# quocdat32461997/ggpm

Hardware: AMD Instinct MI355X
Metric: HierMPNEncoder fwd+bwd target row (SURVEY 8(d): encoder + KL heads + optimizer, tree fixed-point hint on; full depth loops in full_depth_loops, the full VAE fwd+bwd row in vae_step) of BASELINE's molecules/sec VAE fwd+bwd (hidden=300, depth=20, batch=32) (higher is better)
Workload: dtype f32

## Files before the change

### ggpm_amd/_lib.py

```python
from __future__ import annotations

import ctypes
import os
from ctypes import c_char_p, c_double, c_float, c_int, c_size_t, c_void_p, POINTER

from . import build as _build

_LIB = None

GGPM_OK, GGPM_ERR_ARG, GGPM_ERR_LAUNCH, GGPM_ERR_UNSUPPORTED, GGPM_ERR_WORKSPACE = range(5)

P = c_void_p
I = c_int
SIGNATURES = {
    "ggpm_version": (I, []),
    "ggpm_error_string": (c_char_p, [I]),
    "ggpm_padded_hidden": (I, [I]),
    "ggpm_padded_to_csr": (I, [P, I, I, P, P, P]),
    "ggpm_padded_to_csr_pair": (I, [P, I, I, P, P, P, I, I, P, P, P]),
    "ggpm_csr_transpose": (I, [P, P, I, I, P, P, P, P]),
    "ggpm_extract_column": (I, [P, I, I, I, P, P]),
    "ggpm_gemm_workspace_bytes": (c_size_t, [I, I, I]),
    "ggpm_gemm": (I, [I, I, I, I, I, P, I, P, I, P, I, I, P, I, I, I, P, c_size_t, P]),
    "ggpm_gemm_grouped": (I, [I, I, I, I, I, I, P, P]),
# ... 10 lines not shown
    "ggpm_gemm_form_query": (I, [P, P]),
    "ggpm_act_backward": (I, [P, P, I, I, I, I, I, P, P]),
    "ggpm_segment_sum": (I, [P, I, P, P, I, I, P, I, I, I, P]),
    "ggpm_segment_sum_masked": (I, [I, P, I, P, P, I, I, P, I, P, I, I, P, P, I, I, I, P]),
    "ggpm_gather_rows": (I, [P, I, P, I, I, P, I, I, I, P]),
    "ggpm_scatter_rows": (I, [P, I, P, I, I, P, I, I, P]),
    "ggpm_adam_step": (I, [P, P, P, P, c_size_t, c_float, c_float, c_float, c_float, c_float, I, P]),
    "ggpm_flat_sqnorm_workspace_bytes": (c_size_t, [c_size_t]),
    "ggpm_flat_sqnorm_partials": (I, [P, c_size_t, P, c_size_t, P]),
    "ggpm_flat_norm_finish": (I, [P, I, c_float, P, P]),
    "ggpm_adam_step_groups": (I, [P, P, P, P, c_size_t, P, I, P, I, P, I, c_float, P, I, P]),
    "ggpm_onehot": (I, [P, I, I, P, I, I, I, P]),
    "ggpm_embed_graph": (I, [P, I, P, I, I, I, I, P, I, P, I, P]),
    "ggpm_level_bf16_storage": (I, [I, I]),
    "ggpm_level_form_query": (I, [I, I, I, I, I, P, P]),
    "ggpm_gru_backward_stashes": (I, [P, I, I, I, POINTER(c_void_p), POINTER(c_void_p)]),
    "ggpm_lstm_backward_stashes": (I, [P, I, I, I, POINTER(c_void_p), POINTER(c_void_p), POINTER(c_void_p)]),
    "ggpm_sum_slots": (I, [P, I, c_size_t, P, P]),
    "ggpm_gru_pack_floats": (c_size_t, [I]),
    "ggpm_gru_forward": (I, [I, I, I, P, P, P, P, I, P, I, P, P, I, P, P, P, P, P, P, P, P, P, P, I, P, P]),
    "ggpm_gru_backward_workspace_bytes": (c_size_t, [I, I, I]),
    "ggpm_gru_backward": (I, [I, I, I, P, P, I, P, I, P, I, P, P, P, P, P, P, P, P, P, P, P, P, P, P, P,
                              P, I, P, I, P, P, I, P, c_size_t, I, P, P]),
    "ggpm_gru_weight_grads": (I, [I, I, I, P, P, P, P, c_size_t, P, I, P, I, P, P, I, P, P]),
    "ggpm_gru_sparse_forward": (I, [I, I, I, P, P, P, P, P, P, I, P, I, P, P, I, P, P, P, P, P, P, P, P, P, P, I, P, P]),
    "ggpm_gru_sparse_backward": (I, [I, I, I, P, P, P, I, P, I, P, I, P, P, P, P, P, P, P, P, P, P, P, P, P, P, P, P,
                                     P, I, P, I, P, P, I, P, c_size_t, P, P]),
    "ggpm_weight_grads_stacked_workspace_bytes": (c_size_t, [I, I]),
    "ggpm_gru_weight_grads_stacked": (I, [I, I, I, P, P, P, P, P, P, P, I, P, I, P, P, I, P, c_size_t, P]),
    "ggpm_lstm_weight_grads_stacked": (I, [I, I, I, P, P, P, P, P, P, P, I, P, I, P, I, P, I, P, c_size_t, P]),
# ... 122 lines not shown
```

### ggpm_amd/csrc/encoder.hip

```cpp
#include "common.h"
#include "level_call.h"
#include <condition_variable>
#include <cstdlib>
#include <deque>
#include <functional>
#include <mutex>
#include <thread>

namespace {

struct Arena {
    char* base;
    size_t off;
    bool overflow;
    size_t cap;
    template <typename T>
    T* take(size_t n) {
        const size_t bytes = (n * sizeof(T) + 255) & ~(size_t)255;
        T* p = base ? reinterpret_cast<T*>(base + off) : nullptr;
        off += bytes;
        if (base && off > cap) overflow = true;
        return p;
    }
};

struct Csr {
    int32_t *rowptr, *col;
    int rows, ncols, cap;
    int32_t *rowptrT, *colT, *cursor;
};

struct LevelSaved {
    float *X, *Hs, *Cs, *Qs, *St, *wpack, *nei;
    float* hout;
};

struct Saved {
    Csr gpred, gagr, tpred, tagr, tcgr, tsrc, root, motif, attach;
    int32_t *src, *attr0, *motif_id, *attach_id, *iota;
    float *hnode_a, *hmess_a;
    LevelSaved lv[3];
    float *finput_i, *pooled, *hnode_i, *hmess_i, *finput_t, *hnode_t, *hmess_t, *f, *n;
};

struct Dims {
    int H, Hp, He, Hep, depthT, depthG, atom, n_motif, n_attach;
    int N1g, E1g, Kga, Kgb, N1t, E1t, Kta, Ktb, Ktc, B;
    int ld_n, ld_m, ld_t, Ig, It;
    int lstm, nX;
// ... 40 lines not shown
    c.col = A.take<int32_t>(c.cap);
    c.rowptrT = A.take<int32_t>(ncols + 1);
    c.colT = A.take<int32_t>(c.cap);
    c.cursor = A.take<int32_t>(ncols);
}

void take_level(Arena& A, LevelSaved& L, int E1, int N1, int Hp, int H, int depth, bool lstm) {
    const size_t slot = (size_t)E1 * Hp;
    L.X = A.take<float>(cell_gates(lstm).n * slot);
    L.Hs = A.take<float>((size_t)(depth + 1) * slot);
    L.Cs = lstm ? A.take<float>((size_t)(depth + 1) * slot) : nullptr;
    L.Qs = A.take<float>((size_t)depth * slot);
    L.St = A.take<float>((size_t)5 * depth * slot);
    L.wpack = A.take<float>(ggpm_level_pack_floats(lstm, H));
    L.nei = A.take<float>((size_t)N1 * Hp);
}

void layout_saved(Arena& A, const Dims& d, Saved& s) {
    s.lv[0].hout = s.lv[1].hout = s.lv[2].hout = nullptr;
    take_csr(A, s.gpred, d.E1g, d.E1g, d.E1g * d.Kgb);
    take_csr(A, s.gagr, d.N1g, d.E1g, d.N1g * d.Kga);
    take_csr(A, s.tpred, d.E1t, d.E1t, d.E1t * d.Ktb);
    take_csr(A, s.tagr, d.N1t, d.E1t, d.N1t * d.Kta);
    take_csr(A, s.tcgr, d.N1t, d.N1g, d.N1t * d.Ktc);
    s.src = A.take<int32_t>(d.E1t); s.attr0 = A.take<int32_t>(d.E1t);
    s.motif_id = A.take<int32_t>(d.N1t); s.attach_id = A.take<int32_t>(d.N1t);
    const int nio = (d.E1t > d.N1t ? d.E1t : d.N1t) + 1;
    s.iota = A.take<int32_t>(nio > d.B + 1 ? nio : d.B + 1);
    auto take_index = [&](Csr& c, int rows, int ncols) {
        c.rows = rows; c.ncols = ncols; c.cap = rows;
// ... 2 lines not shown
    };
    take_index(s.tsrc, d.E1t, d.N1t);
    take_index(s.root, d.B, d.N1t);
    take_index(s.motif, d.N1t, d.n_motif);
    take_index(s.attach, d.N1t, d.n_attach);
    s.hnode_a = A.take<float>((size_t)d.N1g * d.ld_n);
    s.hmess_a = A.take<float>((size_t)d.E1g * d.ld_m);
    take_level(A, s.lv[0], d.E1t, d.N1t, d.Hp, d.H, d.depthT, d.lstm);
    take_level(A, s.lv[1], d.E1t, d.N1t, d.Hp, d.H, d.depthT, d.lstm);
    take_level(A, s.lv[2], d.E1g, d.N1g, d.Hp, d.H, d.depthG, d.lstm);
    s.finput_i = A.take<float>((size_t)d.N1t * d.Hep); s.pooled = A.take<float>((size_t)d.N1t * d.Hp);
    s.hnode_i = A.take<float>((size_t)d.N1t * d.Hp); s.hmess_i = A.take<float>((size_t)d.E1t * d.ld_t);
    s.finput_t = A.take<float>((size_t)d.N1t * d.Hep);
    s.hnode_t = A.take<float>((size_t)d.N1t * d.Hp); s.hmess_t = A.take<float>((size_t)d.E1t * d.ld_t);
    s.f = A.take<float>((size_t)d.B * d.Hp); s.n = A.take<float>((size_t)d.B * d.Hp);
}

void take_csr_fwd(Arena& A, Csr& c, int rows, int ncols, int cap) {
    c.rows = rows; c.ncols = ncols; c.cap = cap < 1 ? 1 : cap;
    c.rowptr = A.take<int32_t>(rows + 1);
    c.col = A.take<int32_t>(c.cap);
    c.rowptrT = c.colT = c.cursor = nullptr;
}

void layout_infer(Arena& A, const Dims& d, Saved& s) {
    s = Saved{};
    take_csr_fwd(A, s.gpred, d.E1g, d.E1g, d.E1g * d.Kgb);
    take_csr_fwd(A, s.gagr, d.N1g, d.E1g, d.N1g * d.Kga);
    take_csr_fwd(A, s.tpred, d.E1t, d.E1t, d.E1t * d.Ktb);
    take_csr_fwd(A, s.tagr, d.N1t, d.E1t, d.N1t * d.Kta);
// ... 7 lines not shown
    L.X = A.take<float>((size_t)d.nX * slot);
    L.Hs = A.take<float>(2 * slot);
    L.Qs = A.take<float>(2 * slot);
    L.Cs = d.lstm ? A.take<float>(2 * slot) : nullptr;
    L.hout = A.take<float>(slot);
    L.wpack = A.take<float>(ggpm_level_pack_floats(d.lstm, d.H));
    for (int l = 0; l < 3; ++l) {
        s.lv[l] = L;
        s.lv[l].nei = A.take<float>((size_t)(l == 2 ? d.N1g : d.N1t) * d.Hp);
    }
    s.finput_i = A.take<float>((size_t)d.N1t * d.Hep); s.pooled = A.take<float>((size_t)d.N1t * d.Hp);
    s.hnode_i = A.take<float>((size_t)d.N1t * d.Hp); s.hmess_i = A.take<float>((size_t)d.E1t * d.ld_t);
    s.finput_t = A.take<float>((size_t)d.N1t * d.Hep);
    s.hnode_t = A.take<float>((size_t)d.N1t * d.Hp); s.hmess_t = A.take<float>((size_t)d.E1t * d.ld_t);
    s.f = A.take<float>((size_t)d.B * d.Hp); s.n = A.take<float>((size_t)d.B * d.Hp);
}

__global__ void iota_k(int32_t* out, int n) {
    const int i = blockIdx.x * blockDim.x + threadIdx.x;
    if (i < n) out[i] = i;
}

enum { P_EC = 0, P_EI, P_WC, P_BC, P_WI, P_BI, P_WROOT, P_BROOT, P_LEVEL0 };
enum { L_WO = 0, L_BO, L_WZ, L_BZ, L_WR, L_UR, L_BU, L_WH, L_BH, L_COUNT };
enum { Q_WO = 0, Q_BO, Q_WI, Q_BI, Q_WOG, Q_BOG, Q_WU, Q_BU, Q_WF, Q_BF, Q_COUNT };
struct LevelSlots { int count, w[4], b[4], ur, bu, ld[4]; };
constexpr LevelSlots GRU_SLOTS = {L_COUNT, {L_WZ, L_WR, L_WH, -1}, {L_BZ, -1, L_BH, -1}, L_UR, L_BU, {}};
constexpr LevelSlots LSTM_SLOTS = {Q_COUNT, {Q_WI, Q_WOG, Q_WU, Q_WF}, {Q_BI, Q_BOG, Q_BU, Q_BF}, -1, -1, {}};
inline const LevelSlots& level_slots(bool lstm) { return lstm ? LSTM_SLOTS : GRU_SLOTS; }
inline int lwo(const Dims& d, int level) { return P_LEVEL0 + level * level_slots(d.lstm).count + L_WO; }
// ... 173 lines not shown
    return c;
}

int level_forward(const Dims& d, int E1, int N1, int I, int depth, const float* x, int ldx, float* const* P, int level,
                  const Csr& pred, const Csr& agr, LevelSaved& L, ggpm_stream_t s) {
    const int H = d.H, Hp = d.Hp;
    const size_t slot = (size_t)E1 * Hp;
    const int run = run_steps(d, level, depth, E1);
    const LevelTag tag(level);
    ggpm_level_opts o = level_opts(d);
    o.run_depth = run;
    const bool infer = L.hout != nullptr;
    o.h_out = L.hout;
    const int fs = infer ? 0 : fixed_slot(d, level, depth, E1);
    o.fixed_slot = fs;
    const float* result = infer ? L.hout : L.Hs + (size_t)(fs ? fs : depth) * slot;
    const LevelSlots gs = gate_slots(d.lstm, level, I, H);
    const LevelCall c = level_call(d, E1, I, depth, P, gs, pred, L);
    GgpmGemmProblem gp[4];
    for (int k = 0; k < d.nX; ++k)
        gp[k] = {x, ldx, P[gs.w[k]], gs.ld[k], L.X + k * slot, Hp, Hp, gs.b[k] < 0 ? nullptr : P[gs.b[k]], 0, GGPM_ACT_NONE, 0};
    CK(ggpm_gemm_grouped(0, 1, E1, H, I, d.nX, gp, s));
    CK(ggpm_level_forward(c, !infer, &o, s));
    if (!infer) CK(replicate_tail(d, E1, depth, run, level, L, s));
    CK(ggpm_segment_sum(result, Hp, agr.rowptr, agr.col, N1, H, L.nei, Hp, 0, Hp, s));
    return GGPM_OK;
}

int transpose(const Csr& c, const int32_t* col, ggpm_stream_t s) {
    return ggpm_csr_transpose(c.rowptr, col ? col : c.col, c.rows, c.ncols, c.rowptrT, c.colT, c.cursor, s);
// ... 504 lines not shown
```

### ggpm_amd/csrc/level_host.h

```cpp
#pragma once
#include "tile_mma.h"
#include <cstdlib>
#include <type_traits>

namespace {

constexpr size_t GGPM_LDS_LIMIT = 160 * 1024;

template <typename K>
inline void set_lds(K kernel, size_t bytes) { ggpm_set_lds(kernel, bytes); }

inline bool env_no_fuse_b() { static const bool v = ggpm_dev_env("GGPM_NO_FUSE_B") != nullptr; return v; }
inline bool env_adebug() { static const bool v = ggpm_dev_env("GGPM_ADEBUG") != nullptr; return v; }

inline int pick_tg(int E1, int NT) {
    static const char* const tg_env = ggpm_dev_env("GGPM_TG");
    if (const char* e = tg_env) { int v = atoi(e); if (v >= 1 && v <= 64) return v; }
    static const char* const tg_small_env = ggpm_dev_env("GGPM_TG_SMALL");
    if (const char* e = tg_small_env) {
        int v = atoi(e);
        if (v >= 1 && v <= 64 && (E1 + 15) / 16 <= 64) return v < NT ? v : NT;
    }
    static const char* const tg_large_env = ggpm_dev_env("GGPM_TG_LARGE");
    if (const char* e = tg_large_env) {
// ... 18 lines not shown
    static const bool on = [] { const char* e = ggpm_dev_env("GGPM_GATE_SPLIT"); return !e || atoi(e) != 0; }();
    if (!on || rt2) return 0;
    if (dtype != 3 && (!single_group || sparse)) return 0;
    return Cell::mode2_fits(Hp) ? 2 : 0;
}

struct LevelPlan { int tg; bool rt2; int gm; };
template <class Cell>
inline LevelPlan level_plan(const ggpm_level_opts& o, int E1, int Hp, bool sparse) {
    LevelPlan p;
    p.tg = pick_tg(E1, Hp / 16);
    p.rt2 = Cell::use_rt2(o, E1, Hp, sparse);
    p.gm = gate_mode<Cell>(o, Hp, p.rt2, p.tg >= Hp / 16, sparse);
    return p;
}
struct StepLds { int fuse; size_t a, b; };
inline StepLds step_lds(const StepNeed& need, int max_tiles, int Hp, int tg, bool rt2, int gm, bool may_fuse) {
    const int rows = rt2 ? 32 : 16, NT = Hp / 16;
    const bool split = gm == 2;
    const size_t fused = lds_bytes(need.fused, rows, Hp, split);
    StepLds p;
    p.fuse = (!rt2 && may_fuse && ggpm_ceil_div(NT, tg) == 1 && (!max_tiles || NT <= max_tiles) && fused <= GGPM_LDS_LIMIT &&
              !env_no_fuse_b()) ? 1 : 0;
    p.a = p.fuse ? fused : lds_bytes(need.a, rows, Hp, split);
    p.b = lds_bytes(need.b, rows, Hp, split);
    return p;
}
template <class Cell>
inline StepLds fwd_step(int Hp, int tg, bool rt2, int gm, bool with_b) {
    return step_lds(Cell::fwd, 0, Hp, tg, rt2, gm, with_b);
// ... 159 lines not shown
```

### ggpm_amd/csrc/mpn_gru.hip

```cpp
#include "tile_mma.h"
#include "level_host.h"
#include "level_call.h"
#include <cstdlib>
#include <cstdio>

__global__ void ggpm_pack_weight_kernel(GgpmPackArgs a) {
    const int Hp = a.Hp, H = a.H, KC = Hp / 16;
    const int lane = threadIdx.x;
    const int kc = blockIdx.x, t = blockIdx.y, m = blockIdx.z;
    const float* __restrict__ W = a.W[m];
    const int ldw = a.ldw[m];
    const int out = 16 * t + (lane & 15);
    if (a.bf16 == 2) {
        const int KC32 = ggpm_kc32_dev(Hp);
        float x[8];
#pragma unroll
        for (int i = 0; i < 8; ++i) {
            const int k = 32 * kc + 8 * (lane >> 4) + i;
            x[i] = (out < H && k < H) ? (a.transpose ? W[(size_t)k * ldw + out] : W[(size_t)out * ldw + k]) : 0.f;
        }
        uint2 lo[3], hi[3];
        ggpm_split3(make_float4(x[0], x[1], x[2], x[3]), lo[0], lo[1], lo[2]);
        ggpm_split3(make_float4(x[4], x[5], x[6], x[7]), hi[0], hi[1], hi[2]);
        __bf16* dst = reinterpret_cast<__bf16*>(a.dst) + (size_t)m * 2 * ggpm_packed_matrix_floats(Hp, 2);
// ... 60 lines not shown
    float *Hnew, *Qnew;
    float *S, *G, *Z, *M, *R;
    const float *Wz, *Wh, *Ur;
    const float* bu;
    const int32_t *rowptr, *col;
    int ablate;
    const unsigned char* frozen;
    int fuse_b;
    unsigned long long* dbg;
    int bf16;
    int st16;
    int h0_zero;
    float* Hout;
    const float* src_h;
    const int32_t* src_idx;
};

__global__ void pad_bias(const float* __restrict__ b, int H, int Hp, float* __restrict__ out) {
    const int c = blockIdx.x * blockDim.x + threadIdx.x;
    if (c < Hp) out[c] = (c < H) ? b[c] : 0.f;
}

__device__ __forceinline__ float4 one_minus(float4 r) { return make_float4(1.f - r.x, 1.f - r.y, 1.f - r.z, 1.f - r.w); }

template <bool STASH, int GM, int RTT, bool ST16 = false>
__global__ void GGPM_A_BOUNDS gru_fwd_a(GruFwdArgs a) {
    constexpr int ROWS = RTT * 16;
    constexpr bool BF16 = GM == 1, SPLIT = GM == 2;
    static_assert(!SPLIT || RTT == 1, "split operands: one row tile per workgroup");
    static_assert(!ST16 || GM == 1, "bf16 storage goes with bf16 gate products");
    extern __shared__ __attribute__((aligned(16))) float lds[];
// ... 172 lines not shown
        const float* Th = lds + 2 * ROWS * LD;
        for (int tt = wave; tt < NT; tt += GGPM_NWA) {
            const int c = 16 * tt + 4 * (lane >> 4);
            const float4 b = ggpm_ld4(a.bu + c);
            f32x4 acc[1][1];
            ggpm_zero_acc<1, 1>(acc);
            const float* const tiles[1] = {Th};
            const int tn = tt + GGPM_NWA < NT ? tt + GGPM_NWA : -1;
            if constexpr (SPLIT) {
                const __bf16* const imgs[1] = {Ih};
                ggpm_wave_gemm_split<1>(imgs, PLANE, LDH, wps3, KC32, tt, tn, lane, acc, sring3);
            } else if constexpr (BF16) ggpm_wave_gemm_bf16<1, 1>(tiles, LD, wps3, Hp, tt, lane, acc);
            else ggpm_wave_gemm_ring<1, 1>(tiles, LD, wps3, KC, tt, tn, lane, acc, ring3);
            if (row < a.E1) ggpm_stx<ST16>(a.Qnew, (size_t)row * Hp + c, ggpm_f4(acc[0][0]) + b);
        }
    }
}

template <int GM, int RTT, bool ST16 = false>
__global__ void GGPM_A_BOUNDS gru_fwd_b(GruFwdArgs a) {
    constexpr int ROWS = RTT * 16;
    constexpr bool BF16 = GM == 1, SPLIT = GM == 2;
    static_assert(!SPLIT || RTT == 1, "split operands: one row tile per workgroup");
    extern __shared__ __attribute__((aligned(16))) float lds[];
    const int Hp = a.Hp, LD = Hp + 4, KC = Hp / 16, NT = Hp / 16;
    float* Th = lds;
    const int LDH = ggpm_split_ldh(Hp), PLANE = ROWS * LDH, KC32 = ggpm_kc32_dev(Hp);
    __bf16* Ih = reinterpret_cast<__bf16*>(lds);
    const int lane = threadIdx.x & 63;
    const int wave = __builtin_amdgcn_readfirstlane(threadIdx.x >> 6);
// ... 380 lines not shown
        static const int mode = [] { const char* e = ggpm_dev_env("GGPM_RT2"); return e ? atoi(e) : 1; }();
        if (mode == 0 || sparse) return false;
        if (lds_tiles(2, Hp, 32) > GGPM_LDS_LIMIT) return false;
        return mode == 2 || o.prefer_narrow || ggpm_ceil_div(E1, 16) >= GGPM_RT2_MIN_ROW_TILES;
    }
    static bool mode2_fits(int Hp) { return lds_tiles(1, Hp) + 2 * ggpm_split_image_bytes(16, Hp) <= GGPM_LDS_LIMIT; }
    static bool shape_ok(int, int Hp) { return lds_tiles(2, Hp) <= GGPM_LDS_LIMIT; }
};

inline unsigned long long* adebug_stamps(unsigned long long*& buf) {
    if (!env_adebug()) return nullptr;
    if (!buf) (void)hipMalloc(&buf, 64);
    return buf;
}

void launch_fwd(GruFwdArgs a, bool rt2, bool stash, bool with_b, double flops1, hipStream_t s) {
    const StepLds step = fwd_step<GruCell>(a.Hp, a.tg, rt2, a.bf16, with_b);
    a.fuse_b = step.fuse;
    static unsigned long long* dbg_buf = nullptr;
    static int dbg_count = 0;
    a.dbg = adebug_stamps(dbg_buf);
    ggpm_timing_begin(GruCell::timing_base, s, (step.fuse + (a.h0_zero ? 0 : GruCell::gate_products)) * flops1);
    for_variant<GruCell>(a.st16, rt2, a.bf16, [&](auto GM, auto RTT, auto ST16) {
        launch_step(stash ? gru_fwd_a<true, GM, RTT, ST16> : gru_fwd_a<false, GM, RTT, ST16>, a, rt2, step.a, s);
    });
    ggpm_timing_end(GruCell::timing_base, s);
    if (a.dbg && (++dbg_count % 97) == 0) {
        unsigned long long h[7];
        const dim3 grid = step_grid(a, rt2);
        (void)hipStreamSynchronize(s);
        (void)hipMemcpy(h, a.dbg, sizeof(h), hipMemcpyDeviceToHost);
        fprintf(stderr, "[adebug E1=%d grid=%dx%d fuse=%d] gather %.2f barrier %.2f gemm %.2f epilogue %.2f us; wave 15 starts "
                "+%.2f, gathers %.2f\n", a.E1, grid.x, grid.y, a.fuse_b, (h[1] - h[0]) * 0.01, (h[2] - h[1]) * 0.01,
// ... 36 lines not shown
        ggpm_timing_end(GruCell::timing_base + 5, s);
    }
}

}

extern "C" size_t ggpm_gru_pack_floats(int H) {
    const int Hp = ggpm_padded_hidden(H);
    return 3 * ggpm_packed_matrix_slot(Hp) + (size_t)Hp;
}

int ggpm_gru_level_form(int E1, int H, int sparse, int training, const ggpm_level_opts& o, ggpm_level_form* out) {
    return level_form<GruCell>(E1, H, sparse, training, o, out);
}

namespace {
__global__ void sparse_init_state(const float* __restrict__ h_in, const unsigned char* __restrict__ frozen,
                                  float* __restrict__ H0, int Hp) {
    const int c = blockIdx.x * blockDim.x + threadIdx.x;
    const int r = blockIdx.y;
    if (c >= Hp) return;
    H0[(size_t)r * Hp + c] = frozen[r] ? h_in[(size_t)r * Hp + c] : 0.f;
}
}

int gru_forward_impl(const LevelCall& c, int save_for_backward, const ggpm_level_opts& o, ggpm_stream_t stream) {
    GGPM_CLEAR_STALE_ERROR();
    const int E1 = c.rows, H = c.H, depth = c.depth;
    float *Hs = c.Hs, *Qs = c.Qs, *wpack = c.wpack;
    const unsigned char* frozen = c.frozen;
    bool ok = E1 > 0 && H > 0 && depth > 0 && c.bu && c.pred_rowptr && c.pred_col && Hs && Qs && wpack;
    for (int k = 0; k < 3; ++k) ok = ok && c.X[k] && c.W[k];
    for (int k = 0; k < 5; ++k) ok = ok && (c.St[k] || !save_for_backward);
    if (!ok) return GGPM_ERR_ARG;
    const int Hp = ggpm_padded_hidden(H);
    if (!GruCell::shape_ok(E1, Hp)) return GGPM_ERR_UNSUPPORTED;
    hipStream_t s = (hipStream_t)stream;
    const size_t slot = (size_t)E1 * Hp;
    const LevelPlan plan = level_plan<GruCell>(o, E1, Hp, frozen != nullptr);
    const bool rt2 = plan.rt2;
    const int bf16 = plan.gm;
    const size_t mstep = ggpm_packed_matrix_floats(Hp, bf16);
    float* pWz = wpack; float* pWh = wpack + mstep; float* pUr = wpack + 2 * mstep;
    float* pbu = wpack + 3 * ggpm_packed_matrix_slot(Hp);
    {
        GgpmPackArgs pk = {};
        pk.W[0] = c.W[0]; pk.ldw[0] = c.ldw[0]; pk.W[1] = c.W[2]; pk.ldw[1] = c.ldw[2]; pk.W[2] = c.W[1]; pk.ldw[2] = c.ldw[1];
        pk.H = H; pk.Hp = Hp; pk.transpose = 0; pk.dst = wpack; pk.bias = c.bu; pk.bias_out = pbu; pk.bf16 = bf16;
        if (!o.weights_packed) ggpm_launch_pack(pk, 3, s);
    }
    dim3 ig(ggpm_ceil_div(Hp, 256), E1);
    const int tg0 = plan.tg;
    const bool gathered = o.gather_h && o.gather_idx && frozen;
    if (frozen) {
        if (c.h_in != Hs && !gathered) sparse_init_state<<<ig, 256, 0, s>>>(c.h_in, frozen, Hs, Hp);
        GruFwdArgs a0 = {};
// ... 34 lines not shown
            a.R = c.St[4] + (size_t)(t - 1) * slot;
            if (!stash) a.S = a.G = a.Z = a.M = a.R = nullptr;
        } else if (infer) {
            a.Hprev = ggpm_slot_ptr(Hs, (t - 1) & 1, slot, st16); a.Hnew = ggpm_slot_ptr(Hs, t & 1, slot, st16);
            a.Qprev = ggpm_slot_ptr(Qs, (t - 1) & 1, slot, st16); a.Qnew = ggpm_slot_ptr(Qs, t & 1, slot, st16);
            if (t == run_depth) {
                if (st16) a.Hout = o.h_out;
                else a.Hnew = o.h_out;
            }
            a.S = a.G = a.Z = a.M = a.R = nullptr;
        } else {
            a.Hprev = Hs + (size_t)((t - 1) & 1) * slot; a.Hnew = Hs + (size_t)(t & 1) * slot;
            a.Qprev = Qs + (size_t)((t - 1) & 1) * slot; a.Qnew = Qs + (size_t)(t & 1) * slot;
            a.S = a.G = a.Z = a.M = a.R = nullptr;
        }
        launch_fwd(a, rt2, stash, t < depth, flops1, s);
    }
    GGPM_CHECK_LAUNCH();
    return GGPM_OK;
}

#define GRU_FORWARD_OPERANDS(c) \
    c.rows = E1; c.H = H; c.depth = depth; \
    c.X[0] = Xz; c.X[1] = Xr; c.X[2] = Xh; \
    c.W[0] = Wz_h; c.ldw[0] = ld_wz; c.W[1] = Ur; c.ldw[1] = ld_ur; c.W[2] = Wh_h; c.ldw[2] = ld_wh; c.bu = bu; \
    c.pred_rowptr = pred_rowptr; c.pred_col = pred_col; \
    c.Hs = Hs; c.Qs = Qs; c.St[0] = Ss; c.St[1] = Gs; c.St[2] = Zs; c.St[3] = Ms; c.St[4] = Rs; c.wpack = wpack;
extern "C" int ggpm_gru_forward(int E1, int H, int depth, const float* Xz, const float* Xr, const float* Xh,
                                const float* Wz_h, int ld_wz, const float* Ur, int ld_ur, const float* bu,
                                const float* Wh_h, int ld_wh, const int32_t* pred_rowptr,
                                const int32_t* pred_col, float* Hs, float* Qs, float* Ss, float* Gs, float* Zs,
// ... 307 lines not shown
```

### ggpm_amd/functional.py

```python
from __future__ import annotations

import ctypes
import os
import weakref
from typing import List, Optional, Sequence, Tuple

import torch

from . import _dev, _lib
from .nnutils import version_of
from .parallel import grad_view

ACT_NONE, ACT_RELU, ACT_TANH, ACT_SIGMOID = 0, 1, 2, 3


def _stream() -> ctypes.c_void_p:
    return ctypes.c_void_p(torch._C._cuda_getCurrentRawStream(torch._C._cuda_getDevice()))


def _p(t: Optional[torch.Tensor]) -> ctypes.c_void_p:
    return ctypes.c_void_p(0 if t is None else t.data_ptr())


def _need_gpu(*ts: torch.Tensor) -> None:
# ... 559 lines not shown
        v = list(v) if isinstance(v, (list, tuple)) else [v] * 4
        return _I4(*(v + [0] * (4 - len(v))))
    call = GemmCall(GEMM_ENTRIES.index(entry), ta, tb, M, N, count, four(K), four(lda), four(ldb), four(ldc), four(n_pad),
                    four(base_a), four(base_b), four(base_lo), int(ws_bytes is not None), mode, ws_bytes or 0)
    out = GemmForm()
    _lib.check(_lib.load().ggpm_gemm_form_query(ctypes.byref(call), ctypes.byref(out)), "gemm_form_query")
    return out


class LevelOpts(ctypes.Structure):
    _fields_ = [("gate_dtype", ctypes.c_int), ("prefer_narrow", ctypes.c_int), ("weights_packed", ctypes.c_int),
                ("defer_stash", ctypes.c_void_p * 4), ("gather_h", ctypes.c_void_p), ("gather_c", ctypes.c_void_p),
                ("gather_idx", ctypes.c_void_p), ("scatter_h", ctypes.c_void_p), ("scatter_c", ctypes.c_void_p),
                ("scatter_idx", ctypes.c_void_p), ("skip_x_sums", ctypes.c_int), ("run_depth", ctypes.c_int),
                ("lo", ctypes.c_int), ("skip_bias_u", ctypes.c_int), ("skip_sparse_wgrads", ctypes.c_int),
                ("h_out", ctypes.c_void_p), ("c_out", ctypes.c_void_p), ("fixed_slot", ctypes.c_int)]


class LevelForm(ctypes.Structure):
    _fields_ = [("Hp", ctypes.c_int), ("tiles", ctypes.c_int), ("tg", ctypes.c_int), ("groups", ctypes.c_int),
                ("rt2", ctypes.c_int), ("gate_mode", ctypes.c_int), ("st16", ctypes.c_int), ("fuse_fwd", ctypes.c_int),
                ("fuse_bwd", ctypes.c_int), ("lds_fwd_a", ctypes.c_size_t), ("lds_fwd_b", ctypes.c_size_t),
                ("lds_bwd_a", ctypes.c_size_t), ("lds_bwd_b", ctypes.c_size_t)]


def level_form(lstm: bool, E1: int, H: int, sparse: bool = False, training: bool = True, opts: Optional[LevelOpts] = None):
    out = LevelForm()
    rc = _lib.load().ggpm_level_form_query(int(lstm), E1, H, int(sparse), int(training),
                                           None if opts is None else ctypes.byref(opts), ctypes.byref(out))
    if rc == _lib.GGPM_ERR_UNSUPPORTED:
        return None
# ... 885 lines not shown
```

### include/ggpm_hip.h

```cpp
#ifndef GGPM_HIP_H
#define GGPM_HIP_H

#include <stddef.h>
#include <stdint.h>

#ifdef __cplusplus
extern "C" {
#endif

typedef void* ggpm_stream_t;

enum {
    GGPM_OK = 0,
    GGPM_ERR_ARG = 1,
    GGPM_ERR_LAUNCH = 2,
    GGPM_ERR_UNSUPPORTED = 3,
    GGPM_ERR_WORKSPACE = 4
};

enum { GGPM_ACT_NONE = 0, GGPM_ACT_RELU = 1, GGPM_ACT_TANH = 2, GGPM_ACT_SIGMOID = 3 };

int ggpm_version(void);
const char* ggpm_error_string(int code);
int ggpm_padded_hidden(int H);
// ... 147 lines not shown
    float* defer_stash[4];
    const float* gather_h;
    const float* gather_c;
    const int32_t* gather_idx;
    float* scatter_h;
    float* scatter_c;
    const int32_t* scatter_idx;
    int skip_x_sums;
    int run_depth;
    int lo;
    int skip_bias_u;
    int skip_sparse_wgrads;
    float* h_out;
    float* c_out;
    int fixed_slot;
} ggpm_level_opts;

typedef struct ggpm_level_form {
    int Hp, tiles;
    int tg, groups;
    int rt2, gate_mode, st16;
    int fuse_fwd, fuse_bwd;
    size_t lds_fwd_a, lds_fwd_b, lds_bwd_a, lds_bwd_b;
} ggpm_level_form;
int ggpm_level_form_query(int lstm, int E1, int H, int sparse, int training, const ggpm_level_opts* opts,
                          ggpm_level_form* out);

size_t ggpm_gru_pack_floats(int H);
int ggpm_gru_forward(int E1, int H, int depth, const float* Xz, const float* Xr, const float* Xh,
                     const float* Wz_h, int ld_wz, const float* Ur, int ld_ur, const float* bu,
                     const float* Wh_h, int ld_wh, const int32_t* pred_rowptr, const int32_t* pred_col,
// ... 322 lines not shown
```

Baseline: 12260.

## Fuse next-step Ur product into GRU step kernel via K-split partial sums

Adds a K-split path to the GRU message-passing forward for the tree levels. Each column-group block computes a partial product of its freshly produced hidden slice with Ur and writes it to a double-buffered partial buffer. The next step sums these partials while gathering, so the separate per-step Ur GEMM kernel launch is skipped. The cost is extra partial-buffer memory and traffic: every neighbour gather now reads up to five partial arrays, plus workspace in the arena. The path is on by default and can be disabled with an environment variable.

```diff
diff --git a/ggpm_amd/_lib.py b/ggpm_amd/_lib.py
--- a/ggpm_amd/_lib.py
+++ b/ggpm_amd/_lib.py
@@ -48,6 +48,8 @@
     "ggpm_embed_graph": (I, [P, I, P, I, I, I, I, P, I, P, I, P]),
     "ggpm_level_bf16_storage": (I, [I, I]),
     "ggpm_level_form_query": (I, [I, I, I, I, I, P, P]),
+    "ggpm_level_q_part_bytes": (c_size_t, [I, I]),
+    "ggpm_level_ksplit_q": (I, [I, I, I, I, P]),
     "ggpm_gru_backward_stashes": (I, [P, I, I, I, POINTER(c_void_p), POINTER(c_void_p)]),
     "ggpm_lstm_backward_stashes": (I, [P, I, I, I, POINTER(c_void_p), POINTER(c_void_p), POINTER(c_void_p)]),
     "ggpm_sum_slots": (I, [P, I, c_size_t, P, P]),
diff --git a/ggpm_amd/csrc/encoder.hip b/ggpm_amd/csrc/encoder.hip
--- a/ggpm_amd/csrc/encoder.hip
+++ b/ggpm_amd/csrc/encoder.hip
@@ -33,6 +33,8 @@
 struct LevelSaved {
     float *X, *Hs, *Cs, *Qs, *St, *wpack, *nei;
     float* hout;
+    float* qpart;
+    size_t qpart_bytes;
 };
 
 struct Saved {
@@ -103,6 +105,14 @@
     L.St = A.take<float>((size_t)5 * depth * slot);
     L.wpack = A.take<float>(ggpm_level_pack_floats(lstm, H));
     L.nei = A.take<float>((size_t)N1 * Hp);
+}
+
+void take_q_part(Arena& A, const Dims& d, LevelSaved& L) {
+    const ggpm_level_opts o = level_opts(d);
+    L.qpart = nullptr; L.qpart_bytes = 0;
+    if (!ggpm_level_ksplit_q(d.lstm, d.E1t, d.H, 0, &o)) return;
+    L.qpart_bytes = ggpm_level_q_part_bytes(d.E1t, d.H);
+    L.qpart = A.take<float>(L.qpart_bytes / sizeof(float));
 }
 
 void layout_saved(Arena& A, const Dims& d, Saved& s) {
@@ -135,6 +145,8 @@
     s.finput_t = A.take<float>((size_t)d.N1t * d.Hep);
     s.hnode_t = A.take<float>((size_t)d.N1t * d.Hp); s.hmess_t = A.take<float>((size_t)d.E1t * d.ld_t);
     s.f = A.take<float>((size_t)d.B * d.Hp); s.n = A.take<float>((size_t)d.B * d.Hp);
+    for (int l = 0; l < 2; ++l) take_q_part(A, d, s.lv[l]);
+    s.lv[2].qpart = nullptr; s.lv[2].qpart_bytes = 0;
 }
 
 void take_csr_fwd(Arena& A, Csr& c, int rows, int ncols, int cap) {
@@ -172,6 +184,8 @@
     s.finput_t = A.take<float>((size_t)d.N1t * d.Hep);
     s.hnode_t = A.take<float>((size_t)d.N1t * d.Hp); s.hmess_t = A.take<float>((size_t)d.E1t * d.ld_t);
     s.f = A.take<float>((size_t)d.B * d.Hp); s.n = A.take<float>((size_t)d.B * d.Hp);
+    take_q_part(A, d, s.lv[0]);
+    s.lv[1].qpart = s.lv[0].qpart; s.lv[1].qpart_bytes = s.lv[0].qpart_bytes;
 }
 
 __global__ void iota_k(int32_t* out, int n) {
@@ -375,6 +389,7 @@
     o.h_out = L.hout;
     const int fs = infer ? 0 : fixed_slot(d, level, depth, E1);
     o.fixed_slot = fs;
+    o.q_part = L.qpart; o.q_part_bytes = L.qpart_bytes;
     const float* result = infer ? L.hout : L.Hs + (size_t)(fs ? fs : depth) * slot;
     const LevelSlots gs = gate_slots(d.lstm, level, I, H);
     const LevelCall c = level_call(d, E1, I, depth, P, gs, pred, L);
diff --git a/ggpm_amd/csrc/level_host.h b/ggpm_amd/csrc/level_host.h
--- a/ggpm_amd/csrc/level_host.h
+++ b/ggpm_amd/csrc/level_host.h
@@ -56,6 +56,14 @@
     p.gm = gate_mode<Cell>(o, Hp, p.rt2, p.tg >= Hp / 16, sparse);
     return p;
 }
+constexpr int GGPM_KSPLIT_MAX_GROUPS = 5;
+inline bool ksplit_q_form(const LevelPlan& p, int Hp) {
+    static const bool on = [] { const char* e = ggpm_dev_env("GGPM_KSPLIT_Q"); return !e || atoi(e) != 0; }();
+    const int groups = ggpm_ceil_div(Hp / 16, p.tg);
+    return on && p.gm == 0 && !p.rt2 && groups >= 2 && groups <= GGPM_KSPLIT_MAX_GROUPS && p.tg <= 2 * GGPM_NWA;
+}
+inline size_t q_part_floats(int E1, int Hp, int tg) { return (size_t)2 * ggpm_ceil_div(Hp / 16, tg) * E1 * Hp; }
+
 struct StepLds { int fuse; size_t a, b; };
 inline StepLds step_lds(const StepNeed& need, int max_tiles, int Hp, int tg, bool rt2, int gm, bool may_fuse) {
     const int rows = rt2 ? 32 : 16, NT = Hp / 16;
diff --git a/ggpm_amd/csrc/mpn_gru.hip b/ggpm_amd/csrc/mpn_gru.hip
--- a/ggpm_amd/csrc/mpn_gru.hip
+++ b/ggpm_amd/csrc/mpn_gru.hip
@@ -98,7 +98,40 @@
     float* Hout;
     const float* src_h;
     const int32_t* src_idx;
+    float* Qpart_out;
+    const float* Qpart_in;
+    float* Qsum;
+    int groups;
 };
+
+constexpr int GGPM_KS_MAXG = GGPM_KSPLIT_MAX_GROUPS;
+__device__ __forceinline__ void ggpm_slice_head(const float* wp, int KC, int t, int k0, int k1, int lane, f32x4 (&r)[4]) {
+#pragma unroll
+    for (int d = 0; d < 4; ++d)
+        r[d] = *reinterpret_cast<const f32x4*>(wp + ggpm_pack_index(t, min(k0 + d, k1 - 1), KC, lane));
+}
+__device__ __forceinline__ void ggpm_wave_gemm_slice(const float* tile, int LD, const float* wp, int KC, int t, int k0, int k1,
+                                                     int tn, int k0n, int k1n, int lane, f32x4& acc, f32x4 (&head)[4]) {
+    const int boff = (lane & 15) * LD + 4 * (lane >> 4);
+    for (int kb = k0; kb < k1; kb += 4) {
+        f32x4 nxt[4];
+        const bool more = kb + 4 < k1;
+        if (more) ggpm_slice_head(wp, KC, t, kb + 4, k1, lane, nxt);
+        else if (tn >= 0) ggpm_slice_head(wp, KC, tn, k0n, k1n, lane, nxt);
+#pragma unroll
+        for (int d = 0; d < 4; ++d) {
+            if (kb + d < k1) {
+                const f32x4 b = *reinterpret_cast<const f32x4*>(tile + boff + (kb + d) * 16);
+#pragma unroll
+                for (int s = 0; s < 4; ++s) acc = __builtin_amdgcn_mfma_f32_16x16x4f32(head[d][s], b[s], acc, 0, 0, 0);
+            }
+        }
+        if (more || tn >= 0) {
+#pragma unroll
+            for (int d = 0; d < 4; ++d) head[d] = nxt[d];
+        }
+    }
+}
 
 __global__ void pad_bias(const float* __restrict__ b, int H, int Hp, float* __restrict__ out) {
     const int c = blockIdx.x * blockDim.x + threadIdx.x;
@@ -301,6 +334,267 @@
             else ggpm_wave_gemm_ring<1, 1>(tiles, LD, wps3, KC, tt, tn, lane, acc, ring3);
             if (row < a.E1) ggpm_stx<ST16>(a.Qnew, (size_t)row * Hp + c, ggpm_f4(acc[0][0]) + b);
         }
+    }
+}
+
+template <bool STASH>
+__global__ void GGPM_A_BOUNDS gru_fwd_a_ks(GruFwdArgs a) {
+    extern __shared__ __attribute__((aligned(16))) float lds[];
+    const int Hp = a.Hp, LD = Hp + 4, KC = Hp / 16, NT = Hp / 16;
+    float* Ts = lds;
+    float* Tg = lds + 16 * LD;
+    const int lane = threadIdx.x & 63;
+    const int wave = __builtin_amdgcn_readfirstlane(threadIdx.x >> 6);
+    const int rtile = ((int)(blockIdx.x >> 3) / a.groups) * 8 + (int)(blockIdx.x & 7);
+    if (rtile * 16 >= a.E1) return;
+    const int r0 = rtile * 16;
+    const int grp = (int)(blockIdx.x >> 3) % a.groups;
+    const int t = grp * a.tg + wave;
+    const int t_end = min(NT, (grp + 1) * a.tg);
+    const size_t pslot = (size_t)a.E1 * Hp;
+    const bool dbg_on = a.dbg && rtile == 1 && grp == 0 && threadIdx.x == 0;
+    if (dbg_on) a.dbg[0] = wall_clock64();
+
+    for (int lr = wave; lr < 16; lr += GGPM_NWA) {
+        const int row = r0 + lr;
+        GgpmRowList rl;
+        if (a.h0_zero) { rl.lo = 0; rl.n = 0; } else rl = ggpm_row_list(a.rowptr, row, a.E1);
+        const size_t rowo = (size_t)(row < a.E1 ? row : 0) * Hp;
+        if (Hp <= 320) {
+            const int c = lane * 4, tc = 256 + lane;
+            const bool on = c < Hp, ton = tc < Hp;
+            const int cs = on ? c : 0, tcs = ton ? tc : 0;
+            float4 s = ggpm_zero4(), g = ggpm_zero4(), rc = ggpm_zero4();
+            float s1 = 0.f, g1 = 0.f, rc1 = 0.f;
+            const float4 xr = ggpm_ld4(a.Xr + rowo + cs);
+            const float xr1 = a.Xr[rowo + tcs];
+            for (int base = 0; base < rl.n; base += 64) {
+                const int chunk = ggpm_list_chunk(a.col, rl, base, lane);
+                const int m = min(64, rl.n - base);
+                for (int j = 0; j < m; j += 2) {
+                    float4 h[2], qp[2][GGPM_KS_MAXG];
+                    float h1[2], qp1[2][GGPM_KS_MAXG];
+#pragma unroll
+                    for (int u = 0; u < 2; ++u) {
+                        const size_t p = (size_t)ggpm_list_at(chunk, j + u, m) * Hp;
+                        h[u] = ggpm_ld4(a.Hprev + p + cs);
+                        h1[u] = a.Hprev[p + tcs];
+#pragma unroll
+                        for (int gi = 0; gi < GGPM_KS_MAXG; ++gi) {
+                            const float* part = a.Qpart_in + (gi < a.groups ? gi : 0) * pslot + p;
+                            qp[u][gi] = ggpm_ld4(part + cs);
+                            qp1[u][gi] = part[tcs];
+                        }
+                    }
+#pragma unroll
+                    for (int u = 0; u < 2; ++u) {
+                        float4 q = qp[u][0];
+                        float q1 = qp1[u][0];
+#pragma unroll
+                        for (int gi = 1; gi < GGPM_KS_MAXG; ++gi)
+                            if (gi < a.groups) { q = q + qp[u][gi]; q1 = q1 + qp1[u][gi]; }
+                        const float4 r = ggpm_fsigmoid4<false>(xr + q);
+                        const float4 rh = r * h[u];
+                        s = s + h[u];
+                        g = g + rh;
+                        rc = rc + rh * one_minus(r);
+                        const float r1 = ggpm_fsigmoid<false>(xr1 + q1), rh1 = r1 * h1[u];
+                        s1 = s1 + h1[u];
+                        g1 = g1 + rh1;
+                        rc1 = rc1 + rh1 * (1.f - r1);
+                    }
+                }
+            }
+            if (on) {
+                ggpm_st4(Ts + lr * LD + c, s);
+                ggpm_st4(Tg + lr * LD + c, g);
+                if (STASH && row < a.E1 && (c >> 4) / a.tg == grp) {
+                    const size_t o = (size_t)row * Hp + c;
+                    ggpm_st4(a.S + o, s); ggpm_st4(a.G + o, g); ggpm_st4(a.R + o, rc);
+                }
+            }
+            if (ton) {
+                Ts[lr * LD + tc] = s1;
+                Tg[lr * LD + tc] = g1;
+                if (STASH && row < a.E1 && (tc >> 4) / a.tg == grp) {
+                    const size_t o = (size_t)row * Hp + tc;
+                    a.S[o] = s1; a.G[o] = g1; a.R[o] = rc1;
+                }
+            }
+        } else {
+            for (int c0 = 0; c0 < Hp; c0 += 512) {
+                int c[2], cs[2];
+                bool on[2];
+                float4 s[2], g[2], rc[2], xr[2];
+#pragma unroll
+                for (int k = 0; k < 2; ++k) {
+                    c[k] = c0 + 256 * k + lane * 4;
+                    on[k] = c[k] < Hp;
+                    cs[k] = on[k] ? c[k] : 0;
+                    s[k] = ggpm_zero4(); g[k] = ggpm_zero4(); rc[k] = ggpm_zero4();
+                    xr[k] = ggpm_ld4(a.Xr + rowo + cs[k]);
+                }
+                for (int base = 0; base < rl.n; base += 64) {
+                    const int chunk = ggpm_list_chunk(a.col, rl, base, lane);
+                    const int m = min(64, rl.n - base);
+                    for (int j = 0; j < m; ++j) {
+                        const size_t p = (size_t)ggpm_list_at(chunk, j, m) * Hp;
+                        float4 h[2], qp[2][GGPM_KS_MAXG];
+#pragma unroll
+                        for (int k = 0; k < 2; ++k) {
+                            h[k] = ggpm_ld4(a.Hprev + p + cs[k]);
+#pragma unroll
+                            for (int gi = 0; gi < GGPM_KS_MAXG; ++gi)
+                                qp[k][gi] = ggpm_ld4(a.Qpart_in + (gi < a.groups ? gi : 0) * pslot + p + cs[k]);
+                        }
+#pragma unroll
+                        for (int k = 0; k < 2; ++k) {
+                            float4 q = qp[k][0];
+#pragma unroll
+                            for (int gi = 1; gi < GGPM_KS_MAXG; ++gi)
+                                if (gi < a.groups) q = q + qp[k][gi];
+                            const float4 r = ggpm_fsigmoid4<false>(xr[k] + q);
+                            const float4 rh = r * h[k];
+                            s[k] = s[k] + h[k];
+                            g[k] = g[k] + rh;
+                            rc[k] = rc[k] + rh * one_minus(r);
+                        }
+                    }
+                }
+#pragma unroll
+                for (int k = 0; k < 2; ++k) {
+                    if (!on[k]) continue;
+                    ggpm_st4(Ts + lr * LD + c[k], s[k]);
+                    ggpm_st4(Tg + lr * LD + c[k], g[k]);
+                    if (STASH && row < a.E1 && (c[k] >> 4) / a.tg == grp) {
+                        const size_t o = (size_t)row * Hp + c[k];
+                        ggpm_st4(a.S + o, s[k]); ggpm_st4(a.G + o, g[k]); ggpm_st4(a.R + o, rc[k]);
+                    }
+                }
+            }
+        }
+    }
+    if (dbg_on) a.dbg[1] = wall_clock64();
+
+    const bool p2_gemm = !a.h0_zero;
+    const float* const wps2[2] = {a.Wz, a.Wh};
+    GgpmRing<2> ring2;
+    if (p2_gemm && t < t_end) ggpm_ring_prefetch<2>(wps2, KC, t, lane, ring2);
+    ggpm_lds_barrier();
+    if (dbg_on) a.dbg[2] = wall_clock64();
+
+    const int lr = lane & 15, row = r0 + lr;
+    const int k0 = grp * a.tg, k1 = t_end;
+    f32x4 head[4], head2[4];
+    float4 hkeep[2] = {ggpm_zero4(), ggpm_zero4()};
+    auto own_sums = [&](int w0, int nw) {
+        const int n4 = 4 * (k1 - k0);
+        for (int i = (wave - w0) * 64 + lane; i < 16 * n4; i += nw * 64) {
+            const int orow = r0 + i / n4;
+            if (orow >= a.E1) continue;
+            const size_t o = (size_t)orow * Hp + 16 * k0 + 4 * (i % n4);
+            float4 qo[GGPM_KS_MAXG];
+#pragma unroll
+            for (int gi = 0; gi < GGPM_KS_MAXG; ++gi) qo[gi] = ggpm_ld4(a.Qpart_in + (gi < a.groups ? gi : 0) * pslot + o);
+            float4 q = qo[0];
+#pragma unroll
+            for (int gi = 1; gi < GGPM_KS_MAXG; ++gi)
+                if (gi < a.groups) q = q + qo[gi];
+            ggpm_st4(a.Qsum + o, q);
+        }
+    };
+    const bool qsum_on = a.Qsum && a.Qpart_in;
+    const int nown = min(k1 - k0, GGPM_NWA);
+    auto prefetch = [&]() {
+        if (a.Qpart_out) {
+            if (wave < NT) ggpm_slice_head(a.Ur, KC, wave, k0, k1, lane, head);
+            if (wave + GGPM_NWA < NT) ggpm_slice_head(a.Ur, KC, wave + GGPM_NWA, k0, k1, lane, head2);
+        }
+    };
+    auto p2_tile = [&](int tt, float4& keep, bool last) {
+        const int c = 16 * tt + 4 * (lane >> 4);
+        const size_t o = (size_t)(row < a.E1 ? row : 0) * Hp + c;
+        const float4 xz = ggpm_ld4(a.Xz + o), xh = ggpm_ld4(a.Xh + o);
+        f32x4 acc[2][1];
+        ggpm_zero_acc<2, 1>(acc);
+        if (p2_gemm) {
+            const float* const tiles[2] = {Ts, Tg};
+            ggpm_wave_gemm_ring<2, 1>(tiles, LD, wps2, KC, tt, last ? -1 : tt + GGPM_NWA, lane, acc, ring2);
+        }
+        if (last) prefetch();
+        if (dbg_on) a.dbg[3] = wall_clock64();
+        if (row >= a.E1) return;
+        float4 h = ggpm_zero4(), z = ggpm_zero4(), m = ggpm_zero4();
+        if (row != 0) {
+            const float4 s = ggpm_ld4(Ts + lr * LD + c);
+            const float4 pz = ggpm_f4(acc[0][0]) + xz, pm = ggpm_f4(acc[1][0]) + xh;
+            z = ggpm_sigmoid4(pz);
+            m = make_float4(tanhf(pm.x), tanhf(pm.y), tanhf(pm.z), tanhf(pm.w));
+            h = make_float4((1.f - z.x) * s.x + z.x * m.x, (1.f - z.y) * s.y + z.y * m.y,
+                            (1.f - z.z) * s.z + z.z * m.z, (1.f - z.w) * s.w + z.w * m.w);
+        }
+        ggpm_st4(a.Hnew + o, h);
+        keep = h;
+        if (STASH) {
+            ggpm_st4(a.Z + o, z);
+            ggpm_st4(a.M + o, m);
+        }
+    };
+    if (t >= t_end) {
+        prefetch();
+        if (qsum_on) own_sums(nown, GGPM_NWA - nown);
+    } else if (t + GGPM_NWA >= t_end) p2_tile(t, hkeep[0], true);
+    else { p2_tile(t, hkeep[0], false); p2_tile(t + GGPM_NWA, hkeep[1], true); }
+    if (dbg_on) a.dbg[4] = wall_clock64();
+
+    if (a.Qpart_out) {
+        ggpm_lds_barrier();
+        if (t < t_end) ggpm_st4(Tg + lr * LD + 16 * t + 4 * (lane >> 4), hkeep[0]);
+        if (t + GGPM_NWA < t_end) ggpm_st4(Tg + lr * LD + 16 * (t + GGPM_NWA) + 4 * (lane >> 4), hkeep[1]);
+        ggpm_lds_barrier();
+        float* const part = a.Qpart_out + (size_t)grp * pslot;
+        int pi = 0;
+        for (int tt = wave; tt < NT; tt += GGPM_NWA, ++pi) {
+            const int c = 16 * tt + 4 * (lane >> 4);
+            const float4 b = grp == 0 ? ggpm_ld4(a.bu + c) : ggpm_zero4();
+            f32x4 acc = {0.f, 0.f, 0.f, 0.f};
+            if (pi == 1) {
+#pragma unroll
+                for (int d = 0; d < 4; ++d) head[d] = head2[d];
+            }
+            ggpm_wave_gemm_slice(Tg, LD, a.Ur, KC, tt, k0, k1, pi >= 1 && tt + GGPM_NWA < NT ? tt + GGPM_NWA : -1, k0, k1, lane, acc, head);
+            if (row < a.E1) ggpm_st4(part + (size_t)row * Hp + c, grp == 0 ? ggpm_f4(acc) + b : ggpm_f4(acc));
+        }
+    }
+    if (qsum_on && nown == GGPM_NWA) own_sums(0, GGPM_NWA);
+    if (dbg_on) a.dbg[7] = wall_clock64();
+}
+
+__global__ void GGPM_A_BOUNDS gru_fwd_b_ks(GruFwdArgs a) {
+    extern __shared__ __attribute__((aligned(16))) float lds[];
+    const int Hp = a.Hp, LD = Hp + 4, KC = Hp / 16, NT = Hp / 16;
+    float* Th = lds;
+    const int lane = threadIdx.x & 63;
+    const int wave = __builtin_amdgcn_readfirstlane(threadIdx.x >> 6);
+    const int r0 = blockIdx.x * 16;
+    const int grp = blockIdx.y;
+    const int t_end = min(NT, (grp + 1) * a.tg);
+    ggpm_load_rows_to_lds<16, false>(a.Hnew, r0, a.E1, Hp, LD, Th);
+    __syncthreads();
+    const int row = r0 + (lane & 15);
+    for (int tt = grp * a.tg + wave; tt < t_end; tt += GGPM_NWA) {
+        const int c = 16 * tt + 4 * (lane >> 4);
+        const float4 b = ggpm_ld4(a.bu + c);
+        f32x4 head[4];
+        ggpm_slice_head(a.Ur, KC, tt, 0, min(NT, a.tg), lane, head);
+        float4 q = ggpm_zero4();
+        for (int gi = 0; gi < a.groups; ++gi) {
+            const int k0 = gi * a.tg, k1 = min(NT, k0 + a.tg);
+            f32x4 acc = {0.f, 0.f, 0.f, 0.f};
+            ggpm_wave_gemm_slice(Th, LD, a.Ur, KC, tt, k0, k1, gi + 1 < a.groups ? tt : -1, k1, min(NT, k1 + a.tg), lane, acc, head);
+            q = gi == 0 ? ggpm_f4(acc) + b : q + ggpm_f4(acc);
+        }
+        if (row < a.E1) ggpm_st4(a.Qnew + (size_t)row * Hp + c, q);
     }
 }
 
@@ -711,9 +1005,37 @@
     return buf;
 }
 
-void launch_fwd(GruFwdArgs a, bool rt2, bool stash, bool with_b, double flops1, hipStream_t s) {
+inline dim3 ks_grid(const GruFwdArgs& a) { return dim3(8 * ggpm_ceil_div(ggpm_ceil_div(a.E1, 16), 8) * a.groups); }
+
+void launch_fwd(GruFwdArgs a, bool rt2, bool stash, bool with_b, bool ks, double flops1, hipStream_t s) {
     const StepLds step = fwd_step<GruCell>(a.Hp, a.tg, rt2, a.bf16, with_b);
     a.fuse_b = step.fuse;
+    if (ks) {
+        static unsigned long long* ks_dbg_buf = nullptr;
+        static int ks_dbg_count = 0;
+        a.dbg = adebug_stamps(ks_dbg_buf);
+        ggpm_timing_begin(GruCell::timing_base, s, ((a.Qpart_out ? 1 : 0) + (a.h0_zero ? 0 : GruCell::gate_products)) * flops1);
+        {
+            auto kernel = stash ? gru_fwd_a_ks<true> : gru_fwd_a_ks<false>;
+            set_lds(kernel, step.a);
+            kernel<<<ks_grid(a), GGPM_NWA * 64, step.a, s>>>(a);
+        }
+        ggpm_timing_end(GruCell::timing_base, s);
+        if (a.dbg && a.Qpart_in && a.Qpart_out && (++ks_dbg_count % 97) == 0) {
+            unsigned long long h[8];
+            (void)hipStreamSynchronize(s);
+            (void)hipMemcpy(h, a.dbg, sizeof(h), hipMemcpyDeviceToHost);
+            fprintf(stderr, "[adebug ksplit E1=%d groups=%d] gather %.2f barrier %.2f gemm %.2f epilogue %.2f partial q' %.2f us\n",
+                    a.E1, a.groups, (h[1] - h[0]) * 0.01, (h[2] - h[1]) * 0.01, (h[3] - h[2]) * 0.01, (h[4] - h[3]) * 0.01,
+                    (h[7] - h[4]) * 0.01);
+        }
+        if (with_b && !a.Qpart_out) {
+            ggpm_timing_begin(GruCell::timing_base + 4, s, 1 * flops1);
+            launch_step(gru_fwd_b_ks, a, false, step.b, s);
+            ggpm_timing_end(GruCell::timing_base + 4, s);
+        }
+        return;
+    }
     static unsigned long long* dbg_buf = nullptr;
     static int dbg_count = 0;
     a.dbg = adebug_stamps(dbg_buf);
@@ -780,6 +1102,18 @@
     return level_form<GruCell>(E1, H, sparse, training, o, out);
 }
 
+extern "C" size_t ggpm_level_q_part_bytes(int E1, int H) {
+    if (E1 <= 0 || H <= 0) return 0;
+    const int Hp = ggpm_padded_hidden(H);
+    return q_part_floats(E1, Hp, pick_tg(E1, Hp / 16)) * sizeof(float);
+}
+extern "C" int ggpm_level_ksplit_q(int lstm, int E1, int H, int sparse, const ggpm_level_opts* opts) {
+    if (lstm || sparse || E1 <= 0 || H <= 0) return 0;
+    const int Hp = ggpm_padded_hidden(H);
+    if (!GruCell::shape_ok(E1, Hp)) return 0;
+    return ksplit_q_form(level_plan<GruCell>(ggpm_opts_or_default(opts), E1, Hp, false), Hp) ? 1 : 0;
+}
+
 namespace {
 __global__ void sparse_init_state(const float* __restrict__ h_in, const unsigned char* __restrict__ frozen,
                                   float* __restrict__ H0, int Hp) {
@@ -806,6 +1140,9 @@
     const LevelPlan plan = level_plan<GruCell>(o, E1, Hp, frozen != nullptr);
     const bool rt2 = plan.rt2;
     const int bf16 = plan.gm;
+    const bool ks = o.q_part && !frozen && ksplit_q_form(plan, Hp);
+    const size_t qblock = q_part_floats(E1, Hp, plan.tg) / 2;
+    if (ks && o.q_part_bytes < 2 * qblock * sizeof(float)) return GGPM_ERR_WORKSPACE;
     const size_t mstep = ggpm_packed_matrix_floats(Hp, bf16);
     float* pWz = wpack; float* pWh = wpack + mstep; float* pUr = wpack + 2 * mstep;
     float* pbu = wpack + 3 * ggpm_packed_matrix_slot(Hp);
@@ -870,7 +1207,15 @@
             a.Qprev = Qs + (size_t)((t - 1) & 1) * slot; a.Qnew = Qs + (size_t)(t & 1) * slot;
             a.S = a.G = a.Z = a.M = a.R = nullptr;
         }
-        launch_fwd(a, rt2, stash, t < depth, flops1, s);
+        if (ks) {
+            a.groups = ggpm_ceil_div(Hp / 16, tg);
+            if (t < run_depth) a.Qpart_out = o.q_part + (size_t)(t & 1) * qblock;
+            if (t > 1) {
+                a.Qpart_in = o.q_part + (size_t)((t - 1) & 1) * qblock;
+                a.Qsum = save_for_backward ? const_cast<float*>(a.Qprev) : nullptr;
+            }
+        }
+        launch_fwd(a, rt2, stash, t < depth, ks, flops1, s);
     }
     GGPM_CHECK_LAUNCH();
     return GGPM_OK;
diff --git a/ggpm_amd/functional.py b/ggpm_amd/functional.py
--- a/ggpm_amd/functional.py
+++ b/ggpm_amd/functional.py
@@ -597,7 +597,8 @@
                 ("gather_idx", ctypes.c_void_p), ("scatter_h", ctypes.c_void_p), ("scatter_c", ctypes.c_void_p),
                 ("scatter_idx", ctypes.c_void_p), ("skip_x_sums", ctypes.c_int), ("run_depth", ctypes.c_int),
                 ("lo", ctypes.c_int), ("skip_bias_u", ctypes.c_int), ("skip_sparse_wgrads", ctypes.c_int),
-                ("h_out", ctypes.c_void_p), ("c_out", ctypes.c_void_p), ("fixed_slot", ctypes.c_int)]
+                ("h_out", ctypes.c_void_p), ("c_out", ctypes.c_void_p), ("fixed_slot", ctypes.c_int),
+                ("q_part", ctypes.c_void_p), ("q_part_bytes", ctypes.c_size_t)]
 
 
 class LevelForm(ctypes.Structure):
diff --git a/include/ggpm_hip.h b/include/ggpm_hip.h
--- a/include/ggpm_hip.h
+++ b/include/ggpm_hip.h
@@ -185,7 +185,11 @@
     float* h_out;
     float* c_out;
     int fixed_slot;
+    float* q_part;
+    size_t q_part_bytes;
 } ggpm_level_opts;
+size_t ggpm_level_q_part_bytes(int E1, int H);
+int ggpm_level_ksplit_q(int lstm, int E1, int H, int sparse, const ggpm_level_opts* opts);
 
 typedef struct ggpm_level_form {
     int Hp, tiles;
```

Measured after the change: 12480, median of 6. +1.7%, better.
